# patrick-bedkowski/Generative-DNN-for-Physics-Simulations-CERN

Measured on AMD Instinct MI355X. Metric: GAN-step images/sec (44x44 ZDC) at 1/2/4/8 MI355X; conv MFMA util %, higher is better.
Workload: dtype fp32

## Files before the change

generative-dnn-for-physics-simulations-cern_amd/csrc/conv_common.h:

```cpp
#pragma once
#include "common.h"

enum { MODE_FWD = 0, MODE_DGRAD = 1, MODE_WGRAD = 2 };

struct FastDiv {
  uint32_t m;
  int l;
};
static inline FastDiv mkdiv(uint32_t d) {
  FastDiv f;
  f.l = 0;
  while ((1ull << f.l) < d) ++f.l;
  f.m = (uint32_t)(((1ull << 32) * ((1ull << f.l) - d)) / d + 1);
  return f;
}
__device__ __forceinline__ int fdiv(int x, FastDiv f) {
  return (int)((__umulhi((uint32_t)x, f.m) + (uint32_t)x) >> f.l);
}

struct SubPixel {
  int on;
  int ph[4], pw[4];
  int p0[4], q0[4];
  int oh[4], ow[4];
// ... 53 lines not shown
  if (a.d.rows == nullptr || a.d.rows_px <= 0) return 0x7fffffff;
  const int v = __builtin_amdgcn_readfirstlane(a.d.rows[0]) - a.nbase * a.d.rows_px;
  return v < 0 ? 0 : v;
}

__device__ __forceinline__ void conv_live_gemm(ConvArgs& a, int mode) {
  a.mslot = a.M;
  if (a.d.rows == nullptr) return;
  const int nl = conv_live(a), npx = conv_live_px(a);
  if (mode == MODE_WGRAD) a.Kd = min(nl * (a.Kd / a.d.N), npx);
  else a.M = min(nl * (a.M / a.d.N), npx);
}


struct ConvCall {
  float* stats_part = nullptr;
  int64_t stats_floats = 0;
  const es_affine_t* aff = nullptr;
  const void* bnr_x = nullptr;
  const es_norm_t* bnr_nm = nullptr;
  const es_chain_t* bnr_ch = nullptr;
  float* bnr_part = nullptr;
  int64_t bnr_floats = 0;
  float* det_ws = nullptr;
  int64_t det_floats = 0;
  int stats_chunks = 0;
  int bnr_chunks = 0;
  int det_splits = 0;
  int aff_fused = 0;
  int path = 0;
};
enum { PATH_RING = 1, PATH_SPLIT = 2, PATH_SUBPIXEL = 4, PATH_THIN = 8 };

inline int64_t dgrad_rows(const es_conv_desc_t& d, int n) {
  return (int64_t)n * (d.up_h > 0 ? d.H * d.W : d.Hu * d.Wu);
}

int es_f32_split_level();

extern "C" int64_t es_weight_planes_offset(int64_t n);

int es_conv_ring_launch(ConvArgs& a, int mode, ConvCall& call, hipStream_t st);
int es_conv_ring_launch_f32(ConvArgs& a, int mode, ConvCall& call, hipStream_t st);
int64_t es_wgrad_f32_ring_floats(const es_conv_desc_t& d, const int64_t ys[4], const int64_t xs[4]);
int es_wgrad_f32_ring(const es_conv_desc_t& d, const void* dy, const int64_t ys[4], const void* x,
                      const int64_t xs[4], float* dw, float beta, ConvCall& call, hipStream_t st);
// ... 4 lines not shown
```

generative-dnn-for-physics-simulations-cern_amd/csrc/conv_igemm.hip:

```cpp
#include <algorithm>
#include <cstdlib>

#include "conv_common.h"

int es_thin_conv_fwd(const es_conv_desc_t* d, es_dtype_t dt, const void* x, const int64_t xs[4], const void* wk,
                     const float* bias, void* y, es_dtype_t ydt, const int64_t ys[4], ConvCall& call, hipStream_t st);
int es_thin_conv_dgrad(const es_conv_desc_t* d, es_dtype_t dt, const void* dy, const int64_t ys[4],
                       const void* wd, void* dx, es_dtype_t dxdt, const int64_t dxs[4], float beta,
                       ConvCall& call, hipStream_t st);
int es_thin_conv_wgrad(const es_conv_desc_t* d, es_dtype_t dt, const void* dy, const int64_t ys[4], const void* x,
                       const int64_t xs[4], float* dw, ConvCall& call, hipStream_t st);

namespace {


bool g_no_glds = false;

constexpr int KSTEP_BYTES = 128;
constexpr int ROW_BYTES = KSTEP_BYTES + 16;
constexpr int NTHREADS = 256;

template <typename T, int MODE, int BROWS>
struct LdsImg {
  static constexpr bool TR = (MODE == 2) && sizeof(T) == 2;
// ... 1030 lines not shown
}

extern "C" int es_conv2d_dgrad(const es_conv_desc_t* d, es_dtype_t dt, const void* dy,
                               const int64_t ys[4], const void* wd, void* dxu, es_dtype_t dxdt,
                               const int64_t dxs[4], float beta, es_stream_t stream) {
  ConvCall call;
  return tally(d, dt, call, conv_dgrad(d, dt, dy, ys, wd, dxu, dxdt, dxs, beta, call, (hipStream_t)stream));
}

extern "C" int es_conv2d_dgrad_bnred(const es_conv_desc_t* d, es_dtype_t dt, const void* dy, const int64_t ys[4],
                                     const void* wd, void* dx, es_dtype_t dxdt, const int64_t dxs[4],
                                     const void* x, const es_norm_t* nm, const es_chain_t* ch, float* part,
                                     int64_t part_floats, int* chunks, es_stream_t stream) {
  ES_CHECK_ARG(part && chunks && x && nm && ch, "conv dgrad bnred: NULL argument");
  ConvCall call;
  call.bnr_x = x; call.bnr_nm = nm; call.bnr_ch = ch;
  call.bnr_part = part;
  call.bnr_floats = part_floats;
  const int rc = tally(d, dt, call, conv_dgrad(d, dt, dy, ys, wd, dx, dxdt, dxs, 0.f, call, (hipStream_t)stream));
  *chunks = call.bnr_chunks;
  return rc;
}

extern "C" int es_conv2d_wgrad(const es_conv_desc_t* d, es_dtype_t dt, const void* dy,
                               const int64_t ys[4], const void* x, const int64_t xs[4], float* dw,
                               es_stream_t stream) {
  ConvCall call;
  return tally(d, dt, call, conv_wgrad(d, dt, dy, ys, x, xs, dw, call, (hipStream_t)stream));
}

bool g_es_det = false;

namespace {
int64_t generic_det_floats(const es_conv_desc_t* d) {
  const int64_t per = (int64_t)d->K * d->R * d->S * d->C;
  return per * std::max<int64_t>(8, std::min<int64_t>(2048, (1ll << 26) / per));
}

ConvCall det_call(void* ws, int64_t ws_bytes) {
  ConvCall call;
  call.det_ws = (float*)ws;
  call.det_floats = ws_bytes / (int64_t)sizeof(float);
  return call;
}
}

// ... 400 lines not shown
```

generative-dnn-for-physics-simulations-cern_amd/csrc/conv_thin.hip:

```cpp
#include <algorithm>
#include <type_traits>

#include "conv_common.h"

namespace {

constexpr int NT = 256;

template <typename T> struct V16;
template <> struct V16<float> { static constexpr int N = 4; };
template <> struct V16<bf16> { static constexpr int N = 8; };

template <typename T> __device__ __forceinline__ void ld8(const T* p, float* f);
template <> __device__ __forceinline__ void ld8<bf16>(const bf16* p, float* f) {
  const bf16x8 v = *(const bf16x8*)p;
#pragma unroll
  for (int k = 0; k < 8; ++k) f[k] = (float)v[k];
}
template <> __device__ __forceinline__ void ld8<float>(const float* p, float* f) {
  const float4 a = ((const float4*)p)[0], b = ((const float4*)p)[1];
  f[0] = a.x; f[1] = a.y; f[2] = a.z; f[3] = a.w; f[4] = b.x; f[5] = b.y; f[6] = b.z; f[7] = b.w;
}
template <typename T> __device__ __forceinline__ void st8(T* p, const float* f);
template <> __device__ __forceinline__ void st8<bf16>(bf16* p, const float* f) {
// ... 340 lines not shown
      }
      st8<TO>(o, acc[c]);
    } else {
#pragma unroll
      for (int e = 0; e < VN; ++e) {
        float v = acc[c][e];
        if (t.beta != 0.f) v += t.beta * to_f(o[e]);
        o[e] = from_f<TO>(v);
      }
    }
  }
  }
}

struct ThinBnr {
  const void* x;
  const uint8_t* keep;
  const float *mean, *invstd, *gamma, *beta;
  float scale, slope;
  int dfirst, drop;
  float* part;
};

template <typename T, int RS>
__global__ void __launch_bounds__(NT) k1_dgrad_bnred(Thin t, int LP, ThinBnr b) {
  const es_conv_desc_t& d = t.d;
  t.M = thin_m(t);
  __shared__ float wf[1024];
  __shared__ float r1[NT * 8], r2[NT * 8];
  for (int i = threadIdx.x; i < RS * d.C; i += NT) {
    const int c = i / RS, j = i % RS;
    wf[j * d.C + c] = to_f(((const T*)t.w)[i]);
  }
  const int PPB = NT / LP;
  const int l = threadIdx.x % LP;
  float mu[8], is[8], sc[8], sh[8], s1[8], s2[8];
#pragma unroll
  for (int e = 0; e < 8; ++e) {
    const int c = l * 8 + e;
    mu[e] = b.mean[c];
    is[e] = b.invstd[c];
    sc[e] = (b.gamma ? b.gamma[c] : 1.f) * is[e];
    sh[e] = (b.beta ? b.beta[c] : 0.f) - mu[e] * sc[e];
    s1[e] = s2[e] = 0.f;
  }
  __syncthreads();
  const float dsc = b.drop ? b.scale : 1.f;
// ... 11 lines not shown
      const int mc = lv[u] ? m : m0;
      int n, h, w;
      pix3(mc, d.H, d.W, n, h, w);
      const T* dy = (const T*)t.a + n * t.as[0];
      off[u] = n * t.os[0] + h * t.os[2] + w * t.os[3] + l * 8;
      ld8<T>((const T*)b.x + off[u], hv[u]);
      kb[u] = b.drop ? (uint32_t)b.keep[(int64_t)mc * (d.C / 8) + l] : 0xFFu;
#pragma unroll
      for (int e = 0; e < 8; ++e) acc[u][e] = 0.f;
#pragma unroll
      for (int j = 0; j < RS; ++j) {
        const int ph = h + d.pad - j / d.S, pw = w + d.pad - j % d.S;
        const bool ok = ph >= 0 && pw >= 0 && ph < d.P && pw < d.Q;
        const float gv = to_f(dy[ok ? ph * t.as[2] + pw * t.as[3] : 0]);
        const float g = ok ? gv : 0.f;
        const float* wr = wf + j * d.C + l * 8;
#pragma unroll
        for (int e = 0; e < 8; ++e) acc[u][e] += g * wr[e];
      }
    }
#pragma unroll
    for (int u = 0; u < U; ++u) {
      if (!lv[u]) continue;
      st8<T>((T*)t.out + off[u], acc[u]);
#pragma unroll
      for (int e = 0; e < 8; ++e) {
        const float dv = std::is_same<T, bf16>::value ? (float)(bf16)acc[u][e] : acc[u][e], v = hv[u][e];
        const bool keep = (kb[u] >> e) & 1u;
        const float z = v * sc[e] + sh[e];
        const float zs = b.drop && b.dfirst ? z * b.scale : z;
        const float dn = keep ? dv * (zs > 0.f ? 1.f : b.slope) * dsc : 0.f;
        s1[e] += dn;
        s2[e] += dn * ((v - mu[e]) * is[e]);
      }
    }
  }
#pragma unroll
  for (int e = 0; e < 8; ++e) {
    r1[e * NT + threadIdx.x] = s1[e];
    r2[e * NT + threadIdx.x] = s2[e];
  }
  __syncthreads();
  if (threadIdx.x < LP) {
    float* p = b.part + (int64_t)blockIdx.x * 3 * d.C;
#pragma unroll
    for (int e = 0; e < 8; ++e) {
      float a1 = 0.f, a2 = 0.f;
// ... 354 lines not shown
  Thin t{};
  t.d = *d; t.a = dy; t.w = wd; t.out = dx; t.beta = beta;
  for (int i = 0; i < 4; ++i) { t.as[i] = ys[i]; t.os[i] = dxs[i]; }
  t.M = d->N * d->H * d->W;
  const int LP = k1 ? d->C / vn : 1;
  const es_chain_t* ch = call.bnr_ch;
  const es_norm_t* nm = call.bnr_nm;
  const int lp8 = d->C / 8;
  if (k1 && call.bnr_part && call.bnr_x && nm && ch && dt == dxdt && beta == 0.f && (rs == 4 || rs == 9) &&
      pow2(lp8) && lp8 <= 64 && d->C % 8 == 0 &&
      dxs[3] == d->C && dxs[2] == (int64_t)d->W * d->C && dxs[0] == (int64_t)d->H * d->W * d->C &&
      ((uintptr_t)call.bnr_x & 15) == 0 && (ch->act == ES_ACT_LRELU || ch->act == ES_ACT_RELU) &&
      (!ch->drop.enabled || ch->keep)) {
    const dim3 grid(capped(blocks(t.M, NT / lp8), K1_GRID));
    if ((int64_t)grid.x * 3 * d->C <= call.bnr_floats) {
      ThinBnr b{};
      b.x = call.bnr_x; b.keep = ch->keep;
      b.mean = nm->mean; b.invstd = nm->invstd; b.gamma = nm->gamma; b.beta = nm->beta;
      b.drop = ch->drop.enabled != 0;
      b.scale = b.drop ? ch->drop.scale : 1.f;
      b.dfirst = ch->dropout_first;
      b.slope = ch->act == ES_ACT_LRELU ? ch->slope : 0.f;
      b.part = call.bnr_part;
      if (dt == ES_BF16) {
        if (rs == 4) hipLaunchKernelGGL((k1_dgrad_bnred<bf16, 4>), grid, dim3(NT), 0, st, t, lp8, b);
        else hipLaunchKernelGGL((k1_dgrad_bnred<bf16, 9>), grid, dim3(NT), 0, st, t, lp8, b);
      } else {
        if (rs == 4) hipLaunchKernelGGL((k1_dgrad_bnred<float, 4>), grid, dim3(NT), 0, st, t, lp8, b);
        else hipLaunchKernelGGL((k1_dgrad_bnred<float, 9>), grid, dim3(NT), 0, st, t, lp8, b);
      }
      call.bnr_chunks = (int)grid.x;
      return 1;
    }
  }
  if (dt == ES_BF16) {
    if (dxdt == ES_BF16) launch_dgrad<bf16, bf16>(t, rs, LP, st); else launch_dgrad<bf16, float>(t, rs, LP, st);
  } else {
    if (dxdt == ES_BF16) launch_dgrad<float, bf16>(t, rs, LP, st); else launch_dgrad<float, float>(t, rs, LP, st);
  }
  return 1;
}

int es_thin_conv_wgrad(const es_conv_desc_t* d, es_dtype_t dt, const void* dy, const int64_t ys[4], const void* x,
                       const int64_t xs[4], float* dw, ConvCall& call, hipStream_t st) {
  const int rs = d->R * d->S, vn = dt == ES_BF16 ? 8 : 4;
  const bool c1 = c1_ok(d, rs) && ys[1] == 1 && aligned(ys, 8) && pow2(d->K / 8) && d->K / 8 <= 8;
  const bool k1 = k1_ok(d, rs, vn) && xs[1] == 1 && xs[3] == d->C && aligned(xs, vn);
  if (!c1 && !k1) return 0;
  call.path |= PATH_THIN;
  Thin t{};
  t.d = *d; t.a = dy; t.b = x; t.out = dw;
  for (int i = 0; i < 4; ++i) { t.as[i] = ys[i]; t.bs[i] = xs[i]; }
  t.M = d->N * d->P * d->Q;
  t.det = call.det_ws != nullptr;
  const int LP = k1 ? d->C / vn : 1;
  if (dt == ES_BF16) launch_wgrad<bf16>(t, rs, LP, call, st);
  else launch_wgrad<float>(t, rs, LP, call, st);
// ... 3 lines not shown
```

generative-dnn-for-physics-simulations-cern_amd/csrc/norm.hip:

```cpp
#include "common.h"

bool es_fast_dense_nhwc(const es_view_t* v);
int64_t es_fast_part_floats(const es_view_t* v, int G);
int es_fast_norm_stats(const es_view_t* v, int G, es_dtype_t dt, const void* xp, float* part, hipStream_t st);
void es_fast_norm_fwd(const es_view_t* v, int G, es_dtype_t dt, const void* xp, void* yp, const es_norm_t* nm,
                      const es_chain_t* ch, bool keep_ready, hipStream_t st);
void es_fast_keep_bits(const es_view_t* v, const es_chain_t* ch, hipStream_t st);
int es_fast_norm_bwd_reduce(const es_view_t* v, int G, es_dtype_t dt, const void* xp, const void* dyp,
                            const es_norm_t* nm, const es_chain_t* ch, float* part, hipStream_t st);
int es_fast_norm_bwd_apply(const es_view_t* v, int G, es_dtype_t dt, const void* xp, const void* dyp, void* dxp,
                           const es_norm_t* nm, const es_chain_t* ch, const float* a1, const float* a2,
                           float* dsum, float* part, hipStream_t st);

static int fast_kind(const es_view_t* v, int kind, int groups) {
  if (!es_fast_dense_nhwc(v)) return -1;
  if (kind == ES_NORM_BN) return 0;
  if (kind == ES_NORM_GN && groups > 0 && v->c % groups == 0 && v->h * v->w > 1) return groups;
  return -1;
}

static bool same_view(const es_view_t* a, const es_view_t* b) {
  if (a->n != b->n || a->c != b->c || a->h != b->h || a->w != b->w) return false;
  const int dims[4] = {a->n, a->c, a->h, a->w};
  for (int i = 0; i < 4; ++i)
    if (dims[i] > 1 && a->s[i] != b->s[i]) return false;
  return true;
}

namespace {

struct View {
  int n, c, h, w;
  int64_t s[4];
  const int32_t* rows;
  __device__ __forceinline__ int64_t off(int in, int ic, int ih, int iw) const {
// ... 839 lines not shown
                                    const es_view_t* dx, es_dtype_t dxdt, void* dxp, const float* sums_part,
                                    int chunks, float* dgamma, float* dbeta, float* dsum, void* ws,
                                    es_stream_t stream) {
  hipStream_t st = (hipStream_t)stream;
  ES_CHECK_ARG(nm && nm->kind == ES_NORM_BN && sums_part && chunks > 0 && dxp, "norm_act_bwd_sums: bad args");
  ES_CHECK_ARG(dsum == nullptr || x->c <= 1024, "norm_act_bwd_sums: dsum needs C <= 1024");
  const int fk = fast_kind(x, ES_NORM_BN, 1);
  ES_CHECK_ARG(fk == 0 && xdt == dydt && dydt == dxdt && same_view(x, dy) && same_view(x, dx),
               "norm_act_bwd_sums: needs the dense NHWC fast path");
  View xv = mkview(x);
  int cb, cchunks; int64_t rows, per;
  colred_geometry(xv, cb, cchunks, rows, per);
  const int64_t part_floats = std::max<int64_t>((int64_t)cchunks * 3 * x->c, es_fast_part_floats(x, 0));
  float* part = (float*)ws;
  float* g1 = part + part_floats;
  float* g2 = g1 + x->c;
  launch_sums_finalize(st, sums_part, chunks, x->c, mkcnt((float)rows, x), nm->gamma, g1, g2, dbeta, dgamma, 1.f);
  fast_dsum_finalize(x->c, es_fast_norm_bwd_apply(x, 0, xdt, xp, dyp, dxp, nm, ch, g1, g2, dsum, part, st), part,
                     dsum, st);
  ES_CHECK_LAUNCH();
  return ES_OK;
}

extern "C" int64_t es_channel_sum_ws_bytes(const es_view_t* x) {
  View v = mkview(x);
  int cb, chunks; int64_t rows, per;
  colred_geometry(v, cb, chunks, rows, per);
  return (int64_t)chunks * 3 * v.c * sizeof(float);
}

extern "C" int es_channel_sum(const es_view_t* x, es_dtype_t xdt, const void* xp, float* out,
                              float beta, void* ws, es_stream_t stream) {
  hipStream_t st = (hipStream_t)stream;
  BwdIn b = mk_bwdin(x, xdt, xp, nullptr, nullptr);
  int cb, chunks; int64_t rows, per;
  colred_geometry(b.x, cb, chunks, rows, per);
  if (x->c == 1 && rows < (1ll << 31)) {
    const int nb = std::min<int>(chunks, (int)((rows + 255) / 256));
    hipLaunchKernelGGL(sum1_kernel, dim3(nb), dim3(256), 0, st, b, (int)rows, (float*)ws);
    launch_sums_finalize(st, (const float*)ws, nb, 1, mkcnt(1.f), nullptr, (float*)nullptr, (float*)nullptr, out,
                         (float*)nullptr, beta);
    ES_CHECK_LAUNCH();
    return ES_OK;
  }
  hipLaunchKernelGGL(colred_kernel<RED_SUM>, dim3(cb, chunks), dim3(256), 0, st, b, rows, per, (float*)ws);
  launch_sums_finalize(st, (const float*)ws, chunks, x->c, mkcnt(1.f), nullptr, (float*)nullptr, (float*)nullptr, out, (float*)nullptr, beta);
// ... 80 lines not shown
```

generative-dnn-for-physics-simulations-cern_amd/csrc/norm_fast.hip:

```cpp
#include "common.h"

namespace {

typedef unsigned int nt_u32x4 __attribute__((ext_vector_type(4)));
template <typename T> __device__ __forceinline__ void ld8(const T* p, float* f);
template <> __device__ __forceinline__ void ld8<bf16>(const bf16* p, float* f) {
  const bf16x8 v = *(const bf16x8*)p;
#pragma unroll
  for (int k = 0; k < 8; ++k) f[k] = (float)v[k];
}
template <typename T> __device__ __forceinline__ void ld8nt(const T* p, float* f) { ld8<T>(p, f); }
template <> __device__ __forceinline__ void ld8nt<bf16>(const bf16* p, float* f) {
  const nt_u32x4 w = __builtin_nontemporal_load((const nt_u32x4*)p);
#pragma unroll
  for (int k = 0; k < 4; ++k) {
    f[2 * k] = __uint_as_float(w[k] << 16);
    f[2 * k + 1] = __uint_as_float(w[k] & 0xFFFF0000u);
  }
}
template <> __device__ __forceinline__ void ld8<float>(const float* p, float* f) {
  const float4 a = ((const float4*)p)[0], b = ((const float4*)p)[1];
  f[0] = a.x; f[1] = a.y; f[2] = a.z; f[3] = a.w; f[4] = b.x; f[5] = b.y; f[6] = b.z; f[7] = b.w;
}
template <typename T> __device__ __forceinline__ void st8(T* p, const float* f);
// ... 410 lines not shown
      c1[k] = a.a1[si]; c2[k] = a.a2[si];
    }
    const T* __restrict__ x = (const T*)a.x;
    const T* __restrict__ dy = (const T*)a.dy;
    T* __restrict__ dx = (T*)a.out;
    const int ngroups = (g.rlim - g.rbase + 3) >> 2;
    for (int grp = blockIdx.y * g.RGB + g.rg; grp < ngroups; grp += gridDim.y * g.RGB) {
      const int r0 = g.rbase + grp * 4;
      const int nr = min(4, g.rlim - r0);
      float v[4][8], d[4][8];
#pragma unroll
      for (int j = 0; j < 4; ++j) {
        const int rr = r0 + (j < nr ? j : 0);
        ld8nt<T>(x + (int64_t)rr * a.C + g.c0, v[j]);
        ld8nt<T>(dy + (int64_t)rr * a.C + g.c0, d[j]);
      }
      uint32_t keep[4];
      keep_bits<KM>(a, r0, g.c0, keep);
#pragma unroll
      for (int j = 0; j < 4; ++j) {
        if (j >= nr) break;
#pragma unroll
        for (int k = 0; k < 8; ++k) {
          const float xh = (v[j][k] - mu[k]) * is[k];
          const float dn = chain_bwd_t<CH, KM != KM_NONE>(a, xh * ga[k] + be[k], d[j][k], (keep[j] >> k) & 1u);
          d[j][k] = is[k] * (dn * ga[k] - c1[k] - xh * c2[k]);
          acc[k] += d[j][k];
        }
        st8<T>(dx + (int64_t)(r0 + j) * a.C + g.c0, d[j]);
      }
    }
  }
  if (a.dsum) {
    __shared__ float l1[8 * 256];
#pragma unroll
    for (int k = 0; k < 8; ++k) l1[k * 256 + threadIdx.x] = acc[k];
    __syncthreads();
    for (int h = pow2_ceil(g.RGB) >> 1; h > 0; h >>= 1) {
      if (g.active && g.rg < h && g.rg + h < g.RGB) {
        const int o = threadIdx.x + h * g.TCV;
#pragma unroll
        for (int k = 0; k < 8; ++k) {
          acc[k] += l1[k * 256 + o];
          l1[k * 256 + threadIdx.x] = acc[k];
        }
      }
// ... 163 lines not shown

int es_fast_norm_bwd_reduce(const es_view_t* v, int G, es_dtype_t dt, const void* xp, const void* dyp,
                            const es_norm_t* nm, const es_chain_t* ch, float* part, hipStream_t st) {
  dim3 grid; int chunks;
  fast_geometry(v, G, grid, chunks);
  FastArgs a = mk(v, ch, G);
  a.x = xp; a.dy = dyp; a.part = part;
  a.mean = nm->mean; a.invstd = nm->invstd; a.gamma = nm->gamma; a.beta = nm->beta;
  ES_KM_DISPATCH1(a, bn_reduce_fast, dt, grid, st);
  return chunks;
}

int es_fast_norm_bwd_apply(const es_view_t* v, int G, es_dtype_t dt, const void* xp, const void* dyp, void* dxp,
                           const es_norm_t* nm, const es_chain_t* ch, const float* a1, const float* a2,
                           float* dsum, float* part, hipStream_t st) {
  dim3 grid; int chunks;
  fast_geometry(v, G, grid, chunks);
  FastArgs a = mk(v, ch, G);
  a.x = xp; a.dy = dyp; a.out = dxp; a.a1 = a1; a.a2 = a2; a.dsum = dsum; a.part = part;
  a.mean = nm->mean; a.invstd = nm->invstd; a.gamma = nm->gamma; a.beta = nm->beta;
  ES_KM_DISPATCH(a, bn_bwd_apply_fast, dt, grid, st, true);
  return dsum ? (int)(grid.z * grid.y) : 0;
}
```

generative-dnn-for-physics-simulations-cern_amd/expertsim/hip.py:

```python
from __future__ import annotations

import ctypes as C
import os

import numpy as np
import torch

_LIB_PATH = os.environ.get("ES_LIB") or os.path.join(os.path.dirname(os.path.abspath(__file__)), "_lib",
                                                     "libexpertsim_hip.so")
_lib = None

ES_F32, ES_BF16 = 0, 1
ACT_NONE, ACT_RELU, ACT_LRELU = 0, 1, 2
NORM_NONE, NORM_BN, NORM_GN, NORM_LN = 0, 1, 2, 3


class View(C.Structure):
    _fields_ = [("n", C.c_int), ("c", C.c_int), ("h", C.c_int), ("w", C.c_int), ("s", C.c_int64 * 4),
                ("rows", C.c_void_p)]


class Dropout(C.Structure):
    _fields_ = [("seed", C.c_uint64), ("stream", C.c_uint32), ("threshold", C.c_uint32),
                ("scale", C.c_float), ("enabled", C.c_int), ("step_ptr", C.c_void_p), ("step_mul", C.c_int32),
# ... 74 lines not shown
    "es_conv2d_splitk_ws_bytes": (I64, [P, C.c_int]),
    "es_conv2d_fwd_det": (C.c_int, [P, C.c_int, P, P, P, P, P, C.c_int, P, P, I64, P]),
    "es_conv2d_dgrad_det": (C.c_int, [P, C.c_int, P, P, P, P, C.c_int, P, P, I64, P]),
    "es_conv_set_f32_chunk": (C.c_int, [C.c_int]),
    "es_conv_set_f32_split": (C.c_int, [C.c_int]),
    "es_conv_set_wgrad_ws": (C.c_int, [C.c_int]),
    "es_weight_planes_offset": (C.c_int64, [C.c_int64]),
    "es_pack_weight_planes": (C.c_int, [P, C.c_int64, P, P]),
    "es_pack_conv_weights": (C.c_int, [P, C.c_int, P]),
    "es_conv_launch_count": (C.c_int64, []),
    "es_conv_exec_flops": (C.c_int, [C.POINTER(C.c_double), C.c_int]),
    "es_pack_conv_weight": (C.c_int, [P, C.c_int, C.c_int, C.c_int, C.c_int, C.c_int, P, P, P, C.c_int, P]),
    "es_unpack_conv_grad": (C.c_int, [P, C.c_int, C.c_int, C.c_int, C.c_int, P, P, C.c_float, P]),
    "es_unpack_conv_grad_clear": (C.c_int, [P, C.c_int, C.c_int, C.c_int, C.c_int, P, C.c_float, P]),
    "es_norm_stats_ws_bytes": (I64, [P, C.c_int, C.c_int]),
    "es_norm_stats": (C.c_int, [P, C.c_int, P, C.c_int, C.c_int, C.c_float, P, P, P, P, C.c_float, P, P]),
    "es_norm_act_fwd": (C.c_int, [P, C.c_int, P, P, P, C.c_int, P, P, P, C.c_int, P, P]),
    "es_norm_stats_finalize": (C.c_int, [P, C.c_int, C.c_int, C.c_float, P, P, P, P, C.c_float, P]),
    "es_norm_bwd_ws_bytes": (I64, [P, C.c_int, C.c_int]),
    "es_norm_act_bwd": (C.c_int, [P, C.c_int, P, P, P, P, C.c_int, P, P, C.c_int, P, P, C.c_int, P,
                                  C.c_float, P, P, P, P, P]),
    "es_norm_act_bwd_sums": (C.c_int, [P, C.c_int, P, P, P, P, C.c_int, P, P, C.c_int, P, P, C.c_int, P, P, P,
                                       P, P]),
    "es_norm_stats_merge": (C.c_int, [P, C.c_int, C.c_int, P, P]),
    "es_norm_stats_local": (C.c_int, [P, C.c_int, P, P, P, P]),
    "es_norm_bwd_sync": (C.c_int, [C.c_int, P, C.c_int, P, P, P, P, C.c_int, P, P, C.c_int, P, P, C.c_float, P, P,
                                   P, P, P, P]),
    "es_act_fwd": (C.c_int, [P, C.c_int, P, P, P, C.c_int, P, P]),
    "es_dropout_keep_bits": (C.c_int, [P, P, P]),
    "es_channel_sum_ws_bytes": (I64, [P]),
    "es_channel_sum": (C.c_int, [P, C.c_int, P, P, C.c_float, P, P]),
    "es_maxpool_fwd": (C.c_int, [P, C.c_int, P, C.c_int, C.c_int, C.c_int, C.c_int, P, P, P, P]),
    "es_maxpool_bwd": (C.c_int, [P, C.c_int, P, P, C.c_int, C.c_int, C.c_int, C.c_int, P, P, C.c_float, P]),
    "es_dfront_fwd": (C.c_int, [P, P, C.c_int, C.c_int, C.c_int, P, P, P, P, P, C.c_float, C.c_float, P, P, P, P,
                                P]),
    "es_dfront_part_floats": (I64, [C.c_int]),
    "es_dfront_bwd": (C.c_int, [P, P, C.c_int, C.c_int, C.c_int, P, P, P, P, P, C.c_float, C.c_float, P, P, P, P,
                                P, P, P, P, P, P, P, P]),
    "es_dfront2_ok": (C.c_int, [C.c_int, C.c_int, C.c_int, C.c_int]),
    "es_dfront2_part_floats": (I64, [C.c_int]),
    "es_dfront2_save_floats": (I64, [C.c_int, C.c_int, C.c_int, C.c_int]),
    "es_dfront2_fwd": (C.c_int, [P, P, C.c_int, C.c_int, C.c_int, P, P, P, I64, P, P]),
    "es_dfront2_bwd": (C.c_int, [P, P, C.c_int, C.c_int, C.c_int, P, P, P, P, I64, P, P, P, P, P, P, P, P, P, P,
                                 P, P]),
    "es_dfront2_set_probe": (None, [P]),
    "es_dmlp_part_floats": (I64, [C.c_int, C.c_int]),
# ... 240 lines not shown
```

generative-dnn-for-physics-simulations-cern_amd/expertsim/layers.py:

```python
from __future__ import annotations

import ctypes as C
import os
import math

import numpy as np
import torch

from . import hip


class Act:

    __slots__ = ("t", "dims", "strides", "bn_part", "bn_sums", "px", "sample")

    def __init__(self, t: torch.Tensor, dims, strides, sample: bool = True):
        self.px = 0
        self.sample = bool(sample)
        self.bn_part = None
        self.bn_sums = None
        self.t = t
        self.dims = tuple(int(d) for d in dims)
        self.strides = tuple(int(s) for s in strides)

# ... 455 lines not shown
                  nb = int(hip.lib().es_conv2d_splitk_ws_bytes(C.byref(d), 1))
                  wsb = ws(nb, dy.t.device)
                  hip.call("es_conv2d_dgrad_det", C.byref(d), dy.dt, dy.ptr, hip.strides4(dy.strides), hip.ptr(wd),
                           dx.ptr, dx.dt, hip.strides4(dx.strides), hip.ptr(wsb), nb, hip.stream_ptr())
              else:
                  hip.call("es_conv2d_dgrad", C.byref(d), dy.dt, dy.ptr, hip.strides4(dy.strides), hip.ptr(wd),
                         dx.ptr, dx.dt, hip.strides4(dx.strides), float(beta), hip.stream_ptr())
            return dx
        dxu = Act.nhwc(N, Cc, d.Hu, d.Wu, torch.float32, dy.t.device)
        if self._resized(x):
            self._plain_op().dgrad(dy, dxu, dx_dtype=torch.float32, inv_scale=inv_scale, dx=dxu)
        else:
          with _probed(self.label and self.label + ".dgrad"):
            hip.call("es_conv2d_dgrad", C.byref(d), dy.dt, dy.ptr, hip.strides4(dy.strides), hip.ptr(wd),
                     dxu.ptr, dxu.dt, hip.strides4(dxu.strides), 0.0, hip.stream_ptr())
        if dx is None:
            dx = Act.nhwc(N, Cc, H, W, ddt, dy.t.device)
        maps = self.up.device_maps(dy.t.device)
        hip.call("es_upsample_bwd", C.byref(dxu.view), dxu.dt, dxu.ptr, hip.ptr(maps[2]), hip.ptr(maps[3]),
                 hip.ptr(maps[4]), hip.ptr(maps[5]), C.byref(dx.view), dx.dt, dx.ptr, float(beta),
                 hip.stream_ptr())
        return dx

    def wgrad(self, dy: Act, x: Act, dw_out: torch.Tensor = None, db_out: torch.Tensor = None,
              beta=1.0):
        if self._resized(x):
            return self._plain_op().wgrad(dy, self._resize(x), dw_out, db_out, beta)
        d = self.desc(x)
        dev = dy.t.device
        assert dy.t.dtype == x.t.dtype, (dy.t.dtype, x.t.dtype)
        if _DET and dw_out is not None and dw_out.dtype == torch.float32 and dw_out.is_contiguous():
            ys, xs = hip.strides4(dy.strides), hip.strides4(x.strides)
            nb = int(hip.lib().es_conv2d_wgrad_det_ws_bytes(C.byref(d), dy.dt, ys, xs))
            wsb = ws(nb, dev)
            with _probed(self.label and self.label + ".wgrad"):
                hip.call("es_conv2d_wgrad_det", C.byref(d), dy.dt, dy.ptr, ys, x.ptr, xs, hip.ptr(dw_out),
                         float(beta), hip.ptr(wsb), nb, hip.stream_ptr())
            if db_out is not None:
                channel_sum(dy, db_out, beta)
            return dw_out
        direct = (dw_out is not None and float(beta) == 1.0 and (self.R * self.S == 1 or self.C == 1)
                  and dw_out.is_contiguous() and dw_out.dtype == torch.float32)
        if direct:
            dwk = dw_out
        elif dw_out is not None:
            dwk = getattr(self, "_dwk", None)
# ... 398 lines not shown
```

generative-dnn-for-physics-simulations-cern_amd/expertsim/models/neutron/generator.py:

```python
from __future__ import annotations


import contextlib
import ctypes as C

import torch
from torch import nn

from ... import hip
from ...layers import Act, ConvOp, FoldedNorms, NormOp, Upsample, act_bwd, act_fwd, copy_act
from ...utils import philox
from ..base import ExpertModule, build_tree, get_module


SLOPE = 0.1
P_DROP = 0.2


class GeneratorNeutron(ExpertModule):
    base = 13

    READY = ("conv_layers.13.weight", "conv_layers.9.weight", "conv_layers.5.weight", "conv_layers.0.weight",
             "fc2.0.weight", "fc1.0.weight")

    def __init__(self, noise_dim, cond_dim, di_strength, in_strength, **kwargs):
        super().__init__()
        self.name = "Generator-neutron-1-original-architecture"
        self.di_strength = di_strength
        self.in_strength = in_strength
        self.noise_dim, self.cond_dim = int(noise_dim), int(cond_dim)
        k = self.base
        self.image_shape = (4 * k - 8, 4 * k - 8)
        self.fc2_features = 128 * k * k
        build_tree(self, [
            ("fc1.0", lambda: nn.Linear(self.noise_dim + self.cond_dim, 256)),
            ("fc1.1", lambda: nn.BatchNorm1d(256)),
            ("fc2.0", lambda: nn.Linear(256, self.fc2_features)),
            ("fc2.1", lambda: nn.BatchNorm1d(self.fc2_features)),
            ("conv_layers.0", lambda: nn.Conv2d(128, 256, kernel_size=(3, 3))),
# ... 89 lines not shown
        dev = x0_rows.device
        B = x0_rows.shape[0]
        a1, a2, a3, a4, a5 = fold.fold()
        scope = hip.live_rows(B, rows, rows) if rows is not None else contextlib.nullcontext()
        with scope:
            y = copy_act(Act.of(x0_rows), Act.rows(B, self.noise_dim + self.cond_dim, cdt, dev))
            y = o["fc1"].fwd_affine(y, a1, fused=fused)
            y = o["fc2"].fwd_affine(y, a2, fused=fused)
            y = copy_act(Act(y.t, (B, 128, k, k), (F2, k * k, k, 1)), Act.nhwc(B, 128, k, k, cdt, dev))
            y = o["c0"].fwd_affine(y, a3, fused=fused)
            y = o["c5"].fwd_affine(y, a4, fused=fused)
            y = o["c9"].fwd_affine(y, a5, fused=fused)
            return o["c13"].fwd(y, out_dtype=torch.float32)

    def bwd(self, ctx, dimg: Act, ready=None):
        ready = ready or (lambda name: None)
        o = self.ops()
        cdt = self.compute_dtype
        g = lambda n, a: getattr(get_module(self, n), a).grad
        ch = ctx["ch"]
        dh6 = act_bwd(ctx["h6"], hip.chain_struct(hip.ACT_RELU), dimg, dx_dtype=cdt)
        o["c13"].wgrad(dh6, ctx["y5"], g("conv_layers.13", "weight"), g("conv_layers.13", "bias"))
        ready("conv_layers.13.weight")
        dy5 = o["c13"].dgrad(dh6, ctx["y5"], bn_reduce=(o["bn5"], ctx["h5"], ctx["s5"], ch[4]))
        dh5 = o["bn5"].bwd(ctx["h5"], ctx["s5"], ch[4], dy5, dgamma=g("conv_layers.10", "weight"),
                           dbeta=g("conv_layers.10", "bias"), dsum=g("conv_layers.9", "bias"))
        o["c9"].wgrad(dh5, ctx["y4"], g("conv_layers.9", "weight"), None)
        ready("conv_layers.9.weight")
        dy4 = o["c9"].dgrad(dh5, ctx["y4"], bn_reduce=(o["bn4"], ctx["h4"], ctx["s4"], ch[3]))
        dh4 = o["bn4"].bwd(ctx["h4"], ctx["s4"], ch[3], dy4, dgamma=g("conv_layers.6", "weight"),
                           dbeta=g("conv_layers.6", "bias"), dsum=g("conv_layers.5", "bias"))
        o["c5"].wgrad(dh4, ctx["y3"], g("conv_layers.5", "weight"), None)
        ready("conv_layers.5.weight")
        dy3 = o["c5"].dgrad(dh4, ctx["y3"])
        dh3 = o["bn3"].bwd(ctx["h3"], ctx["s3"], ch[2], dy3, dgamma=g("conv_layers.1", "weight"),
                           dbeta=g("conv_layers.1", "bias"), dsum=g("conv_layers.0", "bias"))
        o["c0"].wgrad(dh3, ctx["y2n"], g("conv_layers.0", "weight"), None)
        ready("conv_layers.0.weight")
        dy2n = o["c0"].dgrad(dh3, ctx["y2n"])
        B, k, F2 = dy2n.dims[0], self.base, self.fc2_features
        dy2 = Act.rows(B, F2, cdt, dy2n.t.device)
        copy_act(dy2n, Act(dy2.t, (B, 128, k, k), (F2, k * k, k, 1)))
        dh2 = o["bn2"].bwd(ctx["h2"], ctx["s2"], ch[1], dy2, dgamma=g("fc2.1", "weight"),
                           dbeta=g("fc2.1", "bias"), dsum=g("fc2.0", "bias"))
        o["fc2"].wgrad(dh2, ctx["y1"], g("fc2.0", "weight"), None)
        ready("fc2.0.weight")
        dy1 = o["fc2"].dgrad(dh2, ctx["y1"], dx_dtype=torch.float32)
        dh1 = o["bn1"].bwd(ctx["h1"], ctx["s1"], ch[0], dy1, dx_dtype=cdt, dgamma=g("fc1.1", "weight"),
                           dbeta=g("fc1.1", "bias"), dsum=g("fc1.0", "bias"))
# ... 15 lines not shown
```

include/expertsim_hip.h:

```cpp
#ifndef EXPERTSIM_HIP_H
#define EXPERTSIM_HIP_H

#include <stdint.h>

#ifdef __cplusplus
extern "C" {
#endif

typedef enum { ES_F32 = 0, ES_BF16 = 1 } es_dtype_t;
enum { ES_OK = 0, ES_ERR_ARG = 1, ES_ERR_HIP = 2, ES_ERR_UNSUPPORTED = 3 };
enum { ES_ACT_NONE = 0, ES_ACT_RELU = 1, ES_ACT_LRELU = 2 };
enum { ES_NORM_NONE = 0, ES_NORM_BN = 1, ES_NORM_GN = 2, ES_NORM_LN = 3 };

typedef void* es_stream_t;

typedef struct {
  int n, c, h, w;
  int64_t s[4];
  const int32_t* rows;
} es_view_t;

typedef struct {
  uint64_t seed;
  uint32_t stream;
// ... 113 lines not shown
int es_norm_stats(const es_view_t* x, es_dtype_t xdt, const void* xp, int kind, int groups,
                  float eps, float* mean, float* invstd, float* running_mean, float* running_var,
                  float momentum, void* ws, es_stream_t stream);
int es_norm_stats_finalize(const float* part, int chunks, int C, float eps, float* mean, float* invstd,
                           float* running_mean, float* running_var, float momentum, es_stream_t stream);
int es_norm_act_fwd(const es_view_t* x, es_dtype_t xdt, const es_norm_t* nm, const es_chain_t* ch,
                    const es_view_t* addend, es_dtype_t adt, const void* addend_ptr, const void* xp,
                    const es_view_t* y, es_dtype_t ydt, void* yp, es_stream_t stream);
int64_t es_norm_bwd_ws_bytes(const es_view_t* x, int kind, int groups);
int es_norm_act_bwd(const es_view_t* x, es_dtype_t xdt, const void* xp, const es_norm_t* nm,
                    const es_chain_t* ch, const es_view_t* dy, es_dtype_t dydt, const void* dyp,
                    const es_view_t* act_ref, es_dtype_t rdt, const void* refp,
                    const es_view_t* dx, es_dtype_t dxdt, void* dxp, float beta, float* dgamma,
                    float* dbeta, float* dsum, void* ws, es_stream_t stream);
int es_conv2d_dgrad_bnred(const es_conv_desc_t* d, es_dtype_t dt, const void* dy, const int64_t ys[4],
                          const void* wd, void* dx, es_dtype_t dxdt, const int64_t dxs[4], const void* x,
                          const es_norm_t* nm, const es_chain_t* ch, float* part, int64_t part_floats,
                          int* chunks, es_stream_t stream);

int es_norm_act_bwd_sums(const es_view_t* x, es_dtype_t xdt, const void* xp, const es_norm_t* nm,
                         const es_chain_t* ch, const es_view_t* dy, es_dtype_t dydt, const void* dyp,
                         const es_view_t* dx, es_dtype_t dxdt, void* dxp, const float* sums_part, int chunks,
                         float* dgamma, float* dbeta, float* dsum, void* ws, es_stream_t stream);


int es_norm_stats_merge(const float* part, int chunks, int C, float* out, es_stream_t stream);
int es_norm_stats_local(const es_view_t* x, es_dtype_t xdt, const void* xp, void* ws, float* out,
                        es_stream_t stream);
int es_norm_bwd_sync(int phase, const es_view_t* x, es_dtype_t xdt, const void* xp, const es_norm_t* nm,
                     const es_chain_t* ch, const es_view_t* dy, es_dtype_t dydt, const void* dyp,
                     const es_view_t* dx, es_dtype_t dxdt, void* dxp, float* sums, float cnt,
                     const float* cnt_mul, float* dgamma, float* dbeta, float* dsum, void* ws,
                     es_stream_t stream);

int es_dropout_keep_bits(const es_view_t* x, const es_chain_t* ch, es_stream_t stream);
int es_act_fwd(const es_view_t* x, es_dtype_t xdt, const void* xp, const es_chain_t* ch,
               const es_view_t* y, es_dtype_t ydt, void* yp, es_stream_t stream);

int64_t es_channel_sum_ws_bytes(const es_view_t* x);
int es_channel_sum(const es_view_t* x, es_dtype_t xdt, const void* xp, float* out, float beta,
                   void* ws, es_stream_t stream);

int es_maxpool_fwd(const es_view_t* x, es_dtype_t dt, const void* xp, int kh, int kw, int sh, int sw,
                   const es_view_t* y, void* yp, uint8_t* idx, es_stream_t stream);
int es_maxpool_bwd(const es_view_t* dy, es_dtype_t dt, const void* dyp, const uint8_t* idx, int kh,
                   int kw, int sh, int sw, const es_view_t* dx, void* dxp, float beta,
// ... 151 lines not shown
```

Measured before the change: 23780.

## Recompute thin K=1 conv dgrad inside BN backward apply instead of storing dy

For the last generator layer (a one-output-channel conv feeding batch norm), the dgrad kernel now runs in a no-store mode that only accumulates the BN reduction sums. The BN backward apply kernel then recomputes the conv dgrad on the fly from dy and the weights. This avoids writing and re-reading the full dy5 activation tensor. In exchange, the cheap K=1 conv taps are computed twice, and a guarded fallback to the old path is kept for unsupported shapes.

```diff
diff --git a/generative-dnn-for-physics-simulations-cern_amd/csrc/conv_common.h b/generative-dnn-for-physics-simulations-cern_amd/csrc/conv_common.h
--- a/generative-dnn-for-physics-simulations-cern_amd/csrc/conv_common.h
+++ b/generative-dnn-for-physics-simulations-cern_amd/csrc/conv_common.h
@@ -99,6 +99,7 @@
   const es_chain_t* bnr_ch = nullptr;
   float* bnr_part = nullptr;
   int64_t bnr_floats = 0;
+  bool bnr_nostore = false;
   float* det_ws = nullptr;
   int64_t det_floats = 0;
   int stats_chunks = 0;
diff --git a/generative-dnn-for-physics-simulations-cern_amd/csrc/conv_igemm.hip b/generative-dnn-for-physics-simulations-cern_amd/csrc/conv_igemm.hip
--- a/generative-dnn-for-physics-simulations-cern_amd/csrc/conv_igemm.hip
+++ b/generative-dnn-for-physics-simulations-cern_amd/csrc/conv_igemm.hip
@@ -1076,6 +1076,25 @@
   return rc;
 }
 
+extern "C" int es_conv2d_dgrad_bnsums(const es_conv_desc_t* d, es_dtype_t dt, const void* dy, const int64_t ys[4],
+                                      const void* wd, const es_view_t* x, es_dtype_t xdt, const void* xp,
+                                      const es_norm_t* nm, const es_chain_t* ch, float* part, int64_t part_floats,
+                                      int* chunks, es_stream_t stream) {
+  ES_CHECK_ARG(d && dy && wd && part && chunks && x && xp && nm && ch, "conv dgrad bnsums: NULL argument");
+  if (int e = check_desc(d)) return e;
+  *chunks = 0;
+  if (nm->kind != ES_NORM_BN || x->n != d->N || x->c != d->C || x->h != d->H || x->w != d->W) return ES_OK;
+  ConvCall call;
+  call.bnr_x = xp; call.bnr_nm = nm; call.bnr_ch = ch;
+  call.bnr_part = part;
+  call.bnr_floats = part_floats;
+  call.bnr_nostore = true;
+  if (!es_thin_conv_dgrad(d, dt, dy, ys, wd, nullptr, xdt, x->s, 0.f, call, (hipStream_t)stream)) return ES_OK;
+  ES_CHECK_LAUNCH();
+  *chunks = call.bnr_chunks;
+  return tally(d, dt, call, ES_OK);
+}
+
 extern "C" int es_conv2d_wgrad(const es_conv_desc_t* d, es_dtype_t dt, const void* dy,
                                const int64_t ys[4], const void* x, const int64_t xs[4], float* dw,
                                es_stream_t stream) {
diff --git a/generative-dnn-for-physics-simulations-cern_amd/csrc/conv_thin.hip b/generative-dnn-for-physics-simulations-cern_amd/csrc/conv_thin.hip
--- a/generative-dnn-for-physics-simulations-cern_amd/csrc/conv_thin.hip
+++ b/generative-dnn-for-physics-simulations-cern_amd/csrc/conv_thin.hip
@@ -386,7 +386,7 @@
   float* part;
 };
 
-template <typename T, int RS>
+template <typename T, int RS, bool STORE = true>
 __global__ void __launch_bounds__(NT) k1_dgrad_bnred(Thin t, int LP, ThinBnr b) {
   const es_conv_desc_t& d = t.d;
   t.M = thin_m(t);
@@ -444,7 +444,7 @@
 #pragma unroll
     for (int u = 0; u < U; ++u) {
       if (!lv[u]) continue;
-      st8<T>((T*)t.out + off[u], acc[u]);
+      if constexpr (STORE) st8<T>((T*)t.out + off[u], acc[u]);
 #pragma unroll
       for (int e = 0; e < 8; ++e) {
         const float dv = std::is_same<T, bf16>::value ? (float)(bf16)acc[u][e] : acc[u][e], v = hv[u][e];
@@ -845,7 +845,15 @@
       b.dfirst = ch->dropout_first;
       b.slope = ch->act == ES_ACT_LRELU ? ch->slope : 0.f;
       b.part = call.bnr_part;
-      if (dt == ES_BF16) {
+      if (call.bnr_nostore) {
+        if (dt == ES_BF16) {
+          if (rs == 4) hipLaunchKernelGGL((k1_dgrad_bnred<bf16, 4, false>), grid, dim3(NT), 0, st, t, lp8, b);
+          else hipLaunchKernelGGL((k1_dgrad_bnred<bf16, 9, false>), grid, dim3(NT), 0, st, t, lp8, b);
+        } else {
+          if (rs == 4) hipLaunchKernelGGL((k1_dgrad_bnred<float, 4, false>), grid, dim3(NT), 0, st, t, lp8, b);
+          else hipLaunchKernelGGL((k1_dgrad_bnred<float, 9, false>), grid, dim3(NT), 0, st, t, lp8, b);
+        }
+      } else if (dt == ES_BF16) {
         if (rs == 4) hipLaunchKernelGGL((k1_dgrad_bnred<bf16, 4>), grid, dim3(NT), 0, st, t, lp8, b);
         else hipLaunchKernelGGL((k1_dgrad_bnred<bf16, 9>), grid, dim3(NT), 0, st, t, lp8, b);
       } else {
@@ -856,6 +864,7 @@
       return 1;
     }
   }
+  if (call.bnr_nostore) return 0;
   if (dt == ES_BF16) {
     if (dxdt == ES_BF16) launch_dgrad<bf16, bf16>(t, rs, LP, st); else launch_dgrad<bf16, float>(t, rs, LP, st);
   } else {
diff --git a/generative-dnn-for-physics-simulations-cern_amd/csrc/norm.hip b/generative-dnn-for-physics-simulations-cern_amd/csrc/norm.hip
--- a/generative-dnn-for-physics-simulations-cern_amd/csrc/norm.hip
+++ b/generative-dnn-for-physics-simulations-cern_amd/csrc/norm.hip
@@ -11,6 +11,11 @@
 int es_fast_norm_bwd_apply(const es_view_t* v, int G, es_dtype_t dt, const void* xp, const void* dyp, void* dxp,
                            const es_norm_t* nm, const es_chain_t* ch, const float* a1, const float* a2,
                            float* dsum, float* part, hipStream_t st);
+bool es_fast_apply_k1_ok(const es_view_t* v, const es_chain_t* ch, const es_conv_desc_t* d, const int64_t gs[4]);
+int es_fast_norm_bwd_apply_k1(const es_view_t* v, es_dtype_t dt, const void* xp, void* dxp, const es_norm_t* nm,
+                              const es_chain_t* ch, const float* a1, const float* a2, float* dsum, float* part,
+                              const es_conv_desc_t* d, const void* g, const int64_t gs[4], const void* wd,
+                              hipStream_t st);
 
 static int fast_kind(const es_view_t* v, int kind, int groups) {
   if (!es_fast_dense_nhwc(v)) return -1;
@@ -896,6 +901,31 @@
   return ES_OK;
 }
 
+extern "C" int es_norm_act_bwd_recompute(const es_view_t* x, es_dtype_t xdt, const void* xp, const es_norm_t* nm,
+                                         const es_chain_t* ch, const es_conv_desc_t* d, const void* dy,
+                                         const int64_t ys[4], const void* wd, const es_view_t* dx, void* dxp,
+                                         const float* sums_part, int chunks, float* dgamma, float* dbeta,
+                                         float* dsum, void* ws, es_stream_t stream) {
+  hipStream_t st = (hipStream_t)stream;
+  ES_CHECK_ARG(x && xp && nm && ch && d && dy && ys && wd && dx && dxp && ws, "norm_act_bwd_recompute: NULL argument");
+  ES_CHECK_ARG(nm->kind == ES_NORM_BN && sums_part && chunks > 0, "norm_act_bwd_recompute: bad args");
+  ES_CHECK_ARG(dsum == nullptr || x->c <= 1024, "norm_act_bwd_recompute: dsum needs C <= 1024");
+  ES_CHECK_ARG(fast_kind(x, ES_NORM_BN, 1) == 0 && same_view(x, dx) && es_fast_apply_k1_ok(x, ch, d, ys),
+               "norm_act_bwd_recompute: needs the dense NHWC fast path behind a stride-1 conv with one output channel");
+  View xv = mkview(x);
+  int cb, cchunks; int64_t rows, per;
+  colred_geometry(xv, cb, cchunks, rows, per);
+  const int64_t part_floats = std::max<int64_t>((int64_t)cchunks * 3 * x->c, es_fast_part_floats(x, 0));
+  float* part = (float*)ws;
+  float* g1 = part + part_floats;
+  float* g2 = g1 + x->c;
+  launch_sums_finalize(st, sums_part, chunks, x->c, mkcnt((float)rows, x), nm->gamma, g1, g2, dbeta, dgamma, 1.f);
+  fast_dsum_finalize(x->c, es_fast_norm_bwd_apply_k1(x, xdt, xp, dxp, nm, ch, g1, g2, dsum, part, d, dy, ys, wd, st),
+                     part, dsum, st);
+  ES_CHECK_LAUNCH();
+  return ES_OK;
+}
+
 extern "C" int64_t es_channel_sum_ws_bytes(const es_view_t* x) {
   View v = mkview(x);
   int cb, chunks; int64_t rows, per;
diff --git a/generative-dnn-for-physics-simulations-cern_amd/csrc/norm_fast.hip b/generative-dnn-for-physics-simulations-cern_amd/csrc/norm_fast.hip
--- a/generative-dnn-for-physics-simulations-cern_amd/csrc/norm_fast.hip
+++ b/generative-dnn-for-physics-simulations-cern_amd/csrc/norm_fast.hip
@@ -456,6 +456,103 @@
         if (j >= nr) break;
 #pragma unroll
         for (int k = 0; k < 8; ++k) {
+          const float xh = (v[j][k] - mu[k]) * is[k];
+          const float dn = chain_bwd_t<CH, KM != KM_NONE>(a, xh * ga[k] + be[k], d[j][k], (keep[j] >> k) & 1u);
+          d[j][k] = is[k] * (dn * ga[k] - c1[k] - xh * c2[k]);
+          acc[k] += d[j][k];
+        }
+        st8<T>(dx + (int64_t)(r0 + j) * a.C + g.c0, d[j]);
+      }
+    }
+  }
+  if (a.dsum) {
+    __shared__ float l1[8 * 256];
+#pragma unroll
+    for (int k = 0; k < 8; ++k) l1[k * 256 + threadIdx.x] = acc[k];
+    __syncthreads();
+    for (int h = pow2_ceil(g.RGB) >> 1; h > 0; h >>= 1) {
+      if (g.active && g.rg < h && g.rg + h < g.RGB) {
+        const int o = threadIdx.x + h * g.TCV;
+#pragma unroll
+        for (int k = 0; k < 8; ++k) {
+          acc[k] += l1[k * 256 + o];
+          l1[k * 256 + threadIdx.x] = acc[k];
+        }
+      }
+      __syncthreads();
+    }
+    if (g.active && g.rg == 0) {
+      float* p = a.part + ((int64_t)blockIdx.z * gridDim.y + blockIdx.y) * 3 * a.C + a.C;
+#pragma unroll
+      for (int k = 0; k < 8; ++k) p[g.c0 + k] = acc[k];
+    }
+  }
+}
+
+struct K1Taps {
+  const void* g; int64_t gs0, gs2, gs3;
+  const void* w;
+  int H, W, P, Q, pad, S;
+};
+
+template <typename T, int KMC, int RS>
+__global__ void __launch_bounds__(256) bn_bwd_apply_k1(FastArgs a, K1Taps t) {
+  constexpr int KM = KMC & 15, CH = KMC >> 4;
+  static_assert(KM == KM_NONE || KM == KM_BITS, "the recompute apply reads stored keep bits");
+  const Geo g = geo(a);
+  float acc[8];
+#pragma unroll
+  for (int k = 0; k < 8; ++k) acc[k] = 0.f;
+  if (g.active) {
+    float mu[8], is[8], ga[8], be[8], c1[8], c2[8], wr[RS][8];
+#pragma unroll
+    for (int k = 0; k < 8; ++k) {
+      const int c = g.c0 + k, si = g.sidx(a, c);
+      mu[k] = a.mean[si]; is[k] = a.invstd[si];
+      ga[k] = a.gamma ? a.gamma[c] : 1.f;
+      be[k] = a.beta ? a.beta[c] : 0.f;
+      c1[k] = a.a1[si]; c2[k] = a.a2[si];
+#pragma unroll
+      for (int q = 0; q < RS; ++q) wr[q][k] = to_f(((const T*)t.w)[c * RS + q]);
+    }
+    const T* __restrict__ x = (const T*)a.x;
+    T* __restrict__ dx = (T*)a.out;
+    const int ngroups = (g.rlim - g.rbase + 3) >> 2;
+    for (int grp = blockIdx.y * g.RGB + g.rg; grp < ngroups; grp += gridDim.y * g.RGB) {
+      const int r0 = g.rbase + grp * 4;
+      const int nr = min(4, g.rlim - r0);
+      float v[4][8], d[4][8], gt[4][RS];
+      int n = r0 / a.HW, h = (r0 - n * a.HW) / t.W, w = r0 - n * a.HW - h * t.W;
+      const int n0 = n, h0 = h, w0 = w;
+#pragma unroll
+      for (int j = 0; j < 4; ++j) {
+        const bool in = j < nr;
+        ld8nt<T>(x + (int64_t)(r0 + (in ? j : 0)) * a.C + g.c0, v[j]);
+        const int nj = in ? n : n0, hj = in ? h : h0, wj = in ? w : w0;
+        const T* gn = (const T*)t.g + nj * t.gs0;
+#pragma unroll
+        for (int q = 0; q < RS; ++q) {
+          const int ph = hj + t.pad - q / t.S, pw = wj + t.pad - q % t.S;
+          const bool ok = ph >= 0 && pw >= 0 && ph < t.P && pw < t.Q;
+          const float gv = to_f(gn[ok ? ph * t.gs2 + pw * t.gs3 : 0]);
+          gt[j][q] = ok ? gv : 0.f;
+        }
+        if (++w == t.W) { w = 0; if (++h == t.H) { h = 0; ++n; } }
+      }
+      uint32_t keep[4];
+      keep_bits<KM>(a, r0, g.c0, keep);
+#pragma unroll
+      for (int j = 0; j < 4; ++j) {
+        if (j >= nr) break;
+#pragma unroll
+        for (int k = 0; k < 8; ++k) d[j][k] = 0.f;
+#pragma unroll
+        for (int q = 0; q < RS; ++q)
+#pragma unroll
+          for (int k = 0; k < 8; ++k) d[j][k] = __builtin_fmaf(gt[j][q], wr[q][k], d[j][k]);
+#pragma unroll
+        for (int k = 0; k < 8; ++k) {
+          if constexpr (sizeof(T) == 2) d[j][k] = (float)(bf16)d[j][k];
           const float xh = (v[j][k] - mu[k]) * is[k];
           const float dn = chain_bwd_t<CH, KM != KM_NONE>(a, xh * ga[k] + be[k], d[j][k], (keep[j] >> k) & 1u);
           d[j][k] = is[k] * (dn * ga[k] - c1[k] - xh * c2[k]);
@@ -665,3 +762,48 @@
   ES_KM_DISPATCH(a, bn_bwd_apply_fast, dt, grid, st, true);
   return dsum ? (int)(grid.z * grid.y) : 0;
 }
+
+bool es_fast_apply_k1_ok(const es_view_t* v, const es_chain_t* ch, const es_conv_desc_t* d, const int64_t gs[4]) {
+  const int rs = d->R * d->S;
+  return es_fast_dense_nhwc(v) && ch && (ch->act == ES_ACT_LRELU || ch->act == ES_ACT_RELU) &&
+         (!ch->drop.enabled || ch->keep) && d->K == 1 && d->stride == 1 && d->hmap == nullptr && d->up_h <= 0 &&
+         d->Hu == d->H && d->Wu == d->W && (rs == 4 || rs == 9) && v->n == d->N && v->c == d->C && v->h == d->H &&
+         v->w == d->W && gs != nullptr;
+}
+
+template <typename T, int RS, int KM>
+static void launch_apply_k1(const FastArgs& a, const K1Taps& t, dim3 grid, hipStream_t st) {
+  const int ch = chain_kind(a);
+  if (ch == CH_LRELU_DFIRST)
+    hipLaunchKernelGGL((bn_bwd_apply_k1<T, KM | (CH_LRELU_DFIRST << 4), RS>), grid, dim3(256), 0, st, a, t);
+  else if (ch == CH_LRELU_DLAST)
+    hipLaunchKernelGGL((bn_bwd_apply_k1<T, KM | (CH_LRELU_DLAST << 4), RS>), grid, dim3(256), 0, st, a, t);
+  else
+    hipLaunchKernelGGL((bn_bwd_apply_k1<T, KM, RS>), grid, dim3(256), 0, st, a, t);
+}
+template <typename T>
+static void dispatch_apply_k1(const FastArgs& a, const K1Taps& t, int rs, dim3 grid, hipStream_t st) {
+  const bool bits = keep_mode(a, true) == KM_BITS;
+  if (rs == 4) {
+    if (bits) launch_apply_k1<T, 4, KM_BITS>(a, t, grid, st); else launch_apply_k1<T, 4, KM_NONE>(a, t, grid, st);
+  } else {
+    if (bits) launch_apply_k1<T, 9, KM_BITS>(a, t, grid, st); else launch_apply_k1<T, 9, KM_NONE>(a, t, grid, st);
+  }
+}
+
+int es_fast_norm_bwd_apply_k1(const es_view_t* v, es_dtype_t dt, const void* xp, void* dxp, const es_norm_t* nm,
+                              const es_chain_t* ch, const float* a1, const float* a2, float* dsum, float* part,
+                              const es_conv_desc_t* d, const void* g, const int64_t gs[4], const void* wd,
+                              hipStream_t st) {
+  dim3 grid; int chunks;
+  fast_geometry(v, 0, grid, chunks);
+  FastArgs a = mk(v, ch, 0);
+  a.x = xp; a.out = dxp; a.a1 = a1; a.a2 = a2; a.dsum = dsum; a.part = part;
+  a.mean = nm->mean; a.invstd = nm->invstd; a.gamma = nm->gamma; a.beta = nm->beta;
+  K1Taps t{};
+  t.g = g; t.gs0 = gs[0]; t.gs2 = gs[2]; t.gs3 = gs[3]; t.w = wd;
+  t.H = d->H; t.W = d->W; t.P = d->P; t.Q = d->Q; t.pad = d->pad; t.S = d->S;
+  if (dt == ES_BF16) dispatch_apply_k1<bf16>(a, t, d->R * d->S, grid, st);
+  else dispatch_apply_k1<float>(a, t, d->R * d->S, grid, st);
+  return dsum ? (int)(grid.z * grid.y) : 0;
+}
diff --git a/generative-dnn-for-physics-simulations-cern_amd/expertsim/hip.py b/generative-dnn-for-physics-simulations-cern_amd/expertsim/hip.py
--- a/generative-dnn-for-physics-simulations-cern_amd/expertsim/hip.py
+++ b/generative-dnn-for-physics-simulations-cern_amd/expertsim/hip.py
@@ -120,6 +120,8 @@
                                   C.c_float, P, P, P, P, P]),
     "es_norm_act_bwd_sums": (C.c_int, [P, C.c_int, P, P, P, P, C.c_int, P, P, C.c_int, P, P, C.c_int, P, P, P,
                                        P, P]),
+    "es_conv2d_dgrad_bnsums": (C.c_int, [P, C.c_int, P, P, P, P, C.c_int, P, P, P, P, I64, P, P]),
+    "es_norm_act_bwd_recompute": (C.c_int, [P, C.c_int, P, P, P, P, P, P, P, P, P, P, C.c_int, P, P, P, P, P]),
     "es_norm_stats_merge": (C.c_int, [P, C.c_int, C.c_int, P, P]),
     "es_norm_stats_local": (C.c_int, [P, C.c_int, P, P, P, P]),
     "es_norm_bwd_sync": (C.c_int, [C.c_int, P, C.c_int, P, P, P, P, C.c_int, P, P, C.c_int, P, P, C.c_float, P, P,
diff --git a/generative-dnn-for-physics-simulations-cern_amd/expertsim/layers.py b/generative-dnn-for-physics-simulations-cern_amd/expertsim/layers.py
--- a/generative-dnn-for-physics-simulations-cern_amd/expertsim/layers.py
+++ b/generative-dnn-for-physics-simulations-cern_amd/expertsim/layers.py
@@ -501,6 +501,33 @@
                  hip.stream_ptr())
         return dx
 
+    def dgrad_norm_bwd(self, dy: Act, x: Act, norm: "NormOp", h: Act, stats, chain, dgamma=None, dbeta=None,
+                       dsum=None, inv_scale=None, dh: Act = None):
+        cdt = dy.t.dtype
+        if (self.K != 1 or self.up is not None or _NORM_SYNC is not None or norm.kind != hip.NORM_BN
+                or h.t.dtype != cdt or h.dims != x.dims or (dsum is not None and h.dims[1] > 1024)):
+            return None
+        d = self.desc(x)
+        wd = self.packed(cdt, 1, inv_scale)
+        N, Cc, H, W = x.dims
+        nm = norm.norm_struct(*stats)
+        floats = 3 * Cc * 2048
+        part = torch.empty(floats, dtype=torch.float32, device=dy.t.device)
+        chunks = C.c_int(0)
+        ys = hip.strides4(dy.strides)
+        with _probed(self.label and self.label + ".dgrad"):
+            hip.call("es_conv2d_dgrad_bnsums", C.byref(d), dy.dt, dy.ptr, ys, hip.ptr(wd), C.byref(h.view), h.dt,
+                     h.ptr, C.byref(nm), C.byref(chain), hip.ptr(part), floats, C.byref(chunks), hip.stream_ptr())
+        if chunks.value <= 0:
+            return None
+        if dh is None:
+            dh = h.like_nhwc(cdt)
+        wsb = ws(hip.lib().es_norm_bwd_ws_bytes(C.byref(h.view), norm.kind, norm.groups), h.t.device)
+        hip.call("es_norm_act_bwd_recompute", C.byref(h.view), h.dt, h.ptr, C.byref(nm), C.byref(chain), C.byref(d),
+                 dy.ptr, ys, hip.ptr(wd), C.byref(dh.view), dh.ptr, hip.ptr(part), chunks.value, hip.ptr(dgamma),
+                 hip.ptr(dbeta), hip.ptr(dsum), hip.ptr(wsb), hip.stream_ptr())
+        return dh
+
     def wgrad(self, dy: Act, x: Act, dw_out: torch.Tensor = None, db_out: torch.Tensor = None,
               beta=1.0):
         if self._resized(x):
diff --git a/generative-dnn-for-physics-simulations-cern_amd/expertsim/models/neutron/generator.py b/generative-dnn-for-physics-simulations-cern_amd/expertsim/models/neutron/generator.py
--- a/generative-dnn-for-physics-simulations-cern_amd/expertsim/models/neutron/generator.py
+++ b/generative-dnn-for-physics-simulations-cern_amd/expertsim/models/neutron/generator.py
@@ -3,6 +3,7 @@
 
 import contextlib
 import ctypes as C
+import os
 
 import torch
 from torch import nn
@@ -15,6 +16,8 @@
 
 SLOPE = 0.1
 P_DROP = 0.2
+_THIN_BNRED = os.environ.get("ES_THIN_BNRED", "1") != "0"
+_THIN_RECOMPUTE = os.environ.get("ES_THIN_RECOMPUTE", "1") != "0"
 
 
 class GeneratorNeutron(ExpertModule):
@@ -150,9 +153,15 @@
         dh6 = act_bwd(ctx["h6"], hip.chain_struct(hip.ACT_RELU), dimg, dx_dtype=cdt)
         o["c13"].wgrad(dh6, ctx["y5"], g("conv_layers.13", "weight"), g("conv_layers.13", "bias"))
         ready("conv_layers.13.weight")
-        dy5 = o["c13"].dgrad(dh6, ctx["y5"], bn_reduce=(o["bn5"], ctx["h5"], ctx["s5"], ch[4]))
-        dh5 = o["bn5"].bwd(ctx["h5"], ctx["s5"], ch[4], dy5, dgamma=g("conv_layers.10", "weight"),
-                           dbeta=g("conv_layers.10", "bias"), dsum=g("conv_layers.9", "bias"))
+        bn5g = dict(dgamma=g("conv_layers.10", "weight"), dbeta=g("conv_layers.10", "bias"),
+                    dsum=g("conv_layers.9", "bias"))
+        dh5 = None
+        if _THIN_BNRED and _THIN_RECOMPUTE:
+            dh5 = o["c13"].dgrad_norm_bwd(dh6, ctx["y5"], o["bn5"], ctx["h5"], ctx["s5"], ch[4], **bn5g)
+        if dh5 is None:
+            red = (o["bn5"], ctx["h5"], ctx["s5"], ch[4]) if _THIN_BNRED else None
+            dy5 = o["c13"].dgrad(dh6, ctx["y5"], bn_reduce=red)
+            dh5 = o["bn5"].bwd(ctx["h5"], ctx["s5"], ch[4], dy5, **bn5g)
         o["c9"].wgrad(dh5, ctx["y4"], g("conv_layers.9", "weight"), None)
         ready("conv_layers.9.weight")
         dy4 = o["c9"].dgrad(dh5, ctx["y4"], bn_reduce=(o["bn4"], ctx["h4"], ctx["s4"], ch[3]))
diff --git a/include/expertsim_hip.h b/include/expertsim_hip.h
--- a/include/expertsim_hip.h
+++ b/include/expertsim_hip.h
@@ -159,6 +159,15 @@
                          const es_chain_t* ch, const es_view_t* dy, es_dtype_t dydt, const void* dyp,
                          const es_view_t* dx, es_dtype_t dxdt, void* dxp, const float* sums_part, int chunks,
                          float* dgamma, float* dbeta, float* dsum, void* ws, es_stream_t stream);
+
+int es_conv2d_dgrad_bnsums(const es_conv_desc_t* d, es_dtype_t dt, const void* dy, const int64_t ys[4],
+                           const void* wd, const es_view_t* x, es_dtype_t xdt, const void* xp,
+                           const es_norm_t* nm, const es_chain_t* ch, float* part, int64_t part_floats,
+                           int* chunks, es_stream_t stream);
+int es_norm_act_bwd_recompute(const es_view_t* x, es_dtype_t xdt, const void* xp, const es_norm_t* nm,
+                              const es_chain_t* ch, const es_conv_desc_t* d, const void* dy, const int64_t ys[4],
+                              const void* wd, const es_view_t* dx, void* dxp, const float* sums_part, int chunks,
+                              float* dgamma, float* dbeta, float* dsum, void* ws, es_stream_t stream);
 
 
 int es_norm_stats_merge(const float* part, int chunks, int C, float* out, es_stream_t stream);
```

Result: no change. 24010 (median of 6 runs) (+1.0%).
